# williamyang1991/FRESCO

Measured on AMD Instinct MI355X. Metric: denoising-steps/sec (8-frame batch, 512^2), FRESCO hot-path step, higher is better.
Workload: dtype f16; 1 GPU; cfg2 (BASELINE.json configs[1]): 8 frames 512x512, SD-1.5 decoder shapes, FRESCO attention only (3x up_blocks.2 HW=1024 C=640 + 3x up_blocks.3 HW=4096 C=320 processor calls per step, projections included), 15-step schedule 1x spatial+cf+temporal / 7x cf+temporal / 7x cf; parallelism=single GPU

## Files before the change

fresco_amd/_lib.py:

```python
import ctypes
import os

_HERE = os.path.dirname(os.path.abspath(__file__))
LIB_PATH = os.environ.get("FRESCO_HIP_LIB") or os.path.join(_HERE, "lib", "libfresco_hip.so")

OK = 0
ERRORS = {
    -1: "FRESCO_EINVAL (null pointer / bad size / inconsistent arguments)",
    -2: "FRESCO_EUNSUPPORTED (shape outside what the kernels are built for)",
    -3: "FRESCO_EWORKSPACE (workspace too small)",
    -4: "FRESCO_ELAUNCH (HIP launch failed)",
}
F16, F32, BF16 = 0, 1, 2
VERSION = "0.5.0.2"


class FrescoHipError(RuntimeError):
    pass


_c = ctypes
_vp, _i, _f, _d, _sz, _i64 = _c.c_void_p, _c.c_int, _c.c_float, _c.c_double, _c.c_size_t, _c.c_int64

SIGNATURES = {
    "fresco_version": (_c.c_char_p, []),
    "fresco_last_error": (_c.c_char_p, []),
    "fresco_prof_enable": (_i, [_i]),
    "fresco_prof_disable": (_i, []),
    "fresco_prof_read": (_i, [_i, _vp, _vp, _vp]),
# ... 72 lines not shown
    "fresco_egnet_resize_add": (_i, [_vp] * 5 + [_i] * 7 + [_f, _vp, _vp]),
    "fresco_egnet_saliency": (_i, [_vp, _vp, _vp] + [_i] * 6 + [_vp]),
    "fresco_canny_workspace_bytes": (_sz, [_i, _i, _i]),
    "fresco_canny_classify": (_i, [_vp, _vp, _i, _i, _i, _i, _i, _vp]),
    "fresco_canny_hysteresis": (_i, [_vp, _vp, _vp, _i, _vp, _sz, _i, _i, _i, _vp]),
}

KEYFRAME_SIGNATURES = {
    "keyframe_resize_table_bytes": (_sz, [_i, _i, _i, _i]),
    "keyframe_resize_table": (_i, [_i, _i, _i, _i, _vp, _sz]),
    "keyframe_resize_area_u8": (_i, [_vp, _vp, _vp, _sz, _i, _i, _i, _i, _i, _vp]),
    "keyframe_workspace_bytes": (_sz, [_i, _i, _i]),
    "keyframe_frame_errors": (_i, [_vp, _vp, _vp, _vp, _sz, _i, _i, _i, _vp]),
}

_lib = None


def load():
    global _lib
    if _lib is not None:
        return _lib
    if not os.path.exists(LIB_PATH):
        raise FrescoHipError(
            "fresco_amd: %s is missing -- build it with `python -c 'import __graft_entry__ as g; g.build()'` "
            "or `make -C fresco_amd/csrc`. There is no CPU / eager fallback." % LIB_PATH)
    try:
        lib = ctypes.CDLL(LIB_PATH)
    except OSError as e:
        raise FrescoHipError("fresco_amd: cannot load %s: %s" % (LIB_PATH, e))
    for name, (res, args) in list(SIGNATURES.items()) + list(KEYFRAME_SIGNATURES.items()):
        try:
            fn = getattr(lib, name)
        except AttributeError:
            raise FrescoHipError("fresco_amd: %s does not export %s (stale build?)" % (LIB_PATH, name))
        fn.restype = res
        fn.argtypes = args
    built = lib.fresco_version().decode().split()
    if built[1:2] != [VERSION]:
        raise FrescoHipError("fresco_amd: %s is version %s, this package binds %s (stale build?)"
                             % (LIB_PATH, " ".join(built[1:2]) or "?", VERSION))
    _lib = lib
    return lib


def check(rc, what):
# ... 6 lines not shown
```

fresco_amd/csrc/attn.hip:

```cpp
#include "attn_cfg.h"
#include "lds_dma.h"
#include <type_traits>

namespace fresco {

template <typename T, int D>
__device__ __forceinline__ void kv_pack_body(const T* __restrict__ k, const T* __restrict__ v,
                                             const int32_t* __restrict__ kv_rows, char* __restrict__ img,
                                             float* __restrict__ ktmax, int H, int M, int nT, int64_t group_rows,
                                             int64_t kv_ld) {
    using Cfg = AttnCfg<D>;
    typedef typename Elem<T>::x8 X8;
    const int tile = blockIdx.x, h = blockIdx.y, g = blockIdx.z;
    __shared__ int32_t rows[64];
    __shared__ __attribute__((aligned(16))) T ks[64][D + 8];
    __shared__ __attribute__((aligned(16))) T vs[64][D + 8];

    if (threadIdx.x < 64) {
        const int m = tile * 64 + threadIdx.x;
        int32_t r = -1;
        if (m < M) r = kv_rows ? kv_rows[m] : m;
        rows[threadIdx.x] = r;
    }
    __syncthreads();
// ... 387 lines not shown
                    if (dA + 8 < D) {
                        const u32x2 a = __builtin_bit_cast(u32x2, wa), bb = __builtin_bit_cast(u32x2, wb);
                        const auto s0 = __builtin_amdgcn_permlane32_swap(a[0], bb[0], false, false);
                        const auto s1 = __builtin_amdgcn_permlane32_swap(a[1], bb[1], false, false);
                        u32x4 st;
                        st[0] = s0[0]; st[1] = s1[0]; st[2] = s0[1]; st[3] = s1[1];
                        if (qr < Lq) *reinterpret_cast<u32x4*>(op + dA + hi * 8) = st;
                    } else if (qr < Lq) {
                        *reinterpret_cast<X4*>(op + dA + hi * 4) = wa;
                    }
                }
        }
    }
}

template <int D, int QB>
struct FlashHalves : std::integral_constant<bool, D == 80 && QB == 2> {};

template <typename T, int D, int QB>
__device__ __forceinline__ void flash_body(const T* __restrict__ q, const char* __restrict__ img,
                                           const float* __restrict__ ktmax, T* __restrict__ out, int H, int Lq,
                                           int M, int nT, int batch_per_group, float scale_log2,
                                           float diag_bias_log2, int64_t q_ld, int h, int qblk, int b, int tid) {
    using Cfg = AttnCfg<D>;
    typedef typename Elem<T>::x8 X8;
    constexpr bool FOLD = FoldCfg<T>::ENABLE;
    extern __shared__ __attribute__((aligned(16))) char smem[];
    constexpr int ROWS = 256 * QB;
    const int g = b / batch_per_group;
    const int C = H * D;

    const int lane = tid & 63, wave = tid >> 6;
    const int l31 = lane & 31, hi = lane >> 5;
    const int qrow0 = qblk * ROWS + wave * 32 * QB + l31;
    const int wave_s = __builtin_amdgcn_readfirstlane(wave);
    const int grpB = wave_s >= 4 ? 1 : 0;

    X8 qf[QB][Cfg::NKS];
    float q2[QB];
#pragma unroll
    for (int j = 0; j < QB; ++j) {
        const int qr = qrow0 + 32 * j;
        const T* qp = q + ((int64_t)b * Lq + (qr < Lq ? qr : Lq - 1)) * q_ld + h * D;
        q2[j] = 0.f;
#pragma unroll
        for (int ks = 0; ks < Cfg::NKS; ++ks) {
            const int d0 = ks * 16 + hi * 8;
            X8 t = {0, 0, 0, 0, 0, 0, 0, 0};
            if (d0 < D) t = *reinterpret_cast<const X8*>(qp + d0);
#pragma unroll
            for (int e = 0; e < 8; ++e) q2[j] = fmaf((float)t[e], (float)t[e], q2[j]);
            qf[j][ks] = t;
        }
        q2[j] += __shfl_xor(q2[j], 32, 64);
    }

    float kmax;
    {
        const float* km = ktmax + (int64_t)(g * H + h) * nT;
        float k2 = 0.f;
        for (int i = lane; i < nT; i += 64) k2 = fmaxf(k2, km[i]);
#pragma unroll
        for (int off = 32; off > 0; off >>= 1) k2 = fmaxf(k2, __shfl_xor(k2, off, 64));
        kmax = sqrtf(k2);
// ... 54 lines not shown
#pragma unroll
            for (int r = 0; r < 16; ++r) {
                s[j][0][r] = Cfg::MCOL ? 0.f : negm[j][r];
                s[j][1][r] = Cfg::MCOL ? 0.f : negm[j][r];
            }
#pragma unroll
        for (int ks = 0; ks < Cfg::NKS; ++ks)
#pragma unroll
            for (int kb = 0; kb < 2; ++kb)
#pragma unroll
                for (int j = 0; j < QB; ++j) {
                    s[j][kb] = Elem<T>::mfma32x32x16(kf[kb][ks], qf[j][ks], s[j][kb]);
                }
    };

    ring.stage(0, 3);
    ring.stage(1, 0);
    if (nT > 1) ring.stage(2, 1);
    if (nT > 2) ring.stage(3, 2);
    ring.wait_barrier(nT > 2 ? 2 : (nT > 1 ? 1 : 0));
    {
        X8 kf[2][Cfg::NKS];
        read_k(kf, 3);
        qk(kf);
    }
    __builtin_amdgcn_sched_barrier(0);

    const int need_diag = diag_bias_log2 != 0.f ? 1 : 0;

    int nomax = 0;
    auto step = [&](int u, auto last_c, auto fast_c) __attribute__((always_inline)) {
        constexpr bool LAST = decltype(last_c)::value;
        constexpr bool FAST = decltype(fast_c)::value;
        const int slot = u & 3;
// ... 125 lines not shown
            u = 1;
            if (!need_diag) {
                bool safe = true;
#pragma unroll
                for (int j = 0; j < QB; ++j) safe = safe && (cmul * (qbound[j] - m_run[j]) <= NOMAX_THR);
                nomax = __builtin_amdgcn_readfirstlane((int)__all(safe));
            }
            if (!need_diag)
                for (; u + 3 < nT; ++u) step(u, no_last, fast);
            for (; u < nT - 1; ++u) step(u, no_last, no);
        }
        nomax = 0;
        step(u, yes, no);
    }

    flash_store<T, D, QB>(o, l_run, out, (int64_t)b * Lq, Lq, C, h, qrow0, l31, hi);
}

template <int X>
__device__ __forceinline__ float lane_xor(float v) {
    return __builtin_bit_cast(float, __builtin_amdgcn_ds_swizzle(__builtin_bit_cast(int, v), (X << 10) | 0x1f));
}

template <typename T, int D>
__device__ __forceinline__ void flash_body_halves(const T* __restrict__ q, const char* __restrict__ img,
                                                  const float* __restrict__ ktmax, T* __restrict__ out, int H,
                                                  int Lq, int M, int nT, int batch_per_group, float scale_log2,
                                                  float diag_bias_log2, int64_t q_ld, int h, int qblk, int b) {
    using Cfg = AttnCfg<D>;
    typedef typename Elem<T>::x8 X8;
    constexpr bool FOLD = FoldCfg<T>::ENABLE;
// ... 312 lines not shown
        const int nQblk = (Lq + 256 * QB - 1) / (256 * QB);                                                           \
        const unsigned blk = blockIdx.x;                                                                              \
        const int h = blk % H;                                                                                        \
        const int qblk = (blk / H) % nQblk;                                                                           \
        const int b = blk / (H * nQblk);                                                                              \
        if constexpr (FlashHalves<D, QB>::value)                                                                      \
            flash_body_halves<T, D>(q, img, ktmax, out, H, Lq, M, nT, batch_per_group, scale_log2, diag_bias_log2,     \
                                    q_ld, h, qblk, b);                                                                \
        else                                                                                                          \
            flash_body<T, D, QB>(q, img, ktmax, out, H, Lq, M, nT, batch_per_group, scale_log2, diag_bias_log2, q_ld,  \
                                 h, qblk, b, threadIdx.x);                                                            \
    }
FRESCO_FLASH_KERNEL(attn_flash_kernel, half_t)
FRESCO_FLASH_KERNEL(attn_flash_bf16_kernel, bf16_t)
#undef FRESCO_FLASH_KERNEL

template <typename T, int D, int QB>
static auto flash_kernel_of() {
    if constexpr (std::is_same<T, bf16_t>::value)
        return &attn_flash_bf16_kernel<D, QB>;
    else
        return &attn_flash_kernel<D, QB>;
}
template <typename T, int D>
static auto kv_pack_kernel_of() {
    if constexpr (std::is_same<T, bf16_t>::value)
        return &kv_pack_bf16_kernel<D>;
    else
        return &kv_pack_kernel<D>;
}
// ... 143 lines not shown
    if (workspace_bytes < attn_ws_bytes(n_groups, H, M, D)) return FRESCO_EWORKSPACE;
    hipStream_t st = as_stream(stream);
    char* ws = static_cast<char*>(workspace);
    return with_elem(dtype, [&](auto e) {
        using T = decltype(e);
        const T* qh = static_cast<const T*>(q);
        const T* xh = static_cast<const T*>(x);
        const T* wk = static_cast<const T*>(Wk);
        const T* wv = static_cast<const T*>(Wv);
        T* oh = static_cast<T*>(out);
        if (D == 40)
            return launch_kvproj_attn<T, 320, 40>(qh, xh, x_ld, x_rows, wk, wv, oh, ws, B, H, Lq, n_groups, M, scale, q_ld, st);
        return launch_kvproj_attn<T, 640, 80>(qh, xh, x_ld, x_rows, wk, wv, oh, ws, B, H, Lq, n_groups, M, scale, q_ld, st);
    });
}
```

fresco_amd/csrc/common.hip:

```cpp
#include "common.h"
#include <string.h>
#include <atomic>
#include <map>
#include <mutex>
#include <utility>

namespace fresco {
static thread_local char g_last_error[256] = "";
void set_last_error(hipError_t e) {
    const char* s = hipGetErrorString(e);
    strncpy(g_last_error, s ? s : "unknown HIP error", sizeof(g_last_error) - 1);
    g_last_error[sizeof(g_last_error) - 1] = 0;
}

static std::mutex g_lds_mu;
static std::map<std::pair<const void*, int>, int> g_lds;

int allow_dyn_lds(const void* fn, int bytes) {
    int dev = 0;
    hipError_t e = hipGetDevice(&dev);
    if (e == hipSuccess) {
        std::lock_guard<std::mutex> lock(g_lds_mu);
        int& allowed = g_lds[{fn, dev}];
        if (bytes <= allowed) return FRESCO_OK;
// ... 79 lines not shown
    using namespace fresco;
    int n = g_prof_n < max_records ? g_prof_n : max_records;
    for (int i = 0; i < n; ++i) {
        (void)hipEventSynchronize(g_prof[i].e1);
        float t = 0.f;
        (void)hipEventElapsedTime(&t, g_prof[i].e0, g_prof[i].e1);
        if (tags) tags[i] = g_prof[i].tag;
        if (dims)
            for (int j = 0; j < 4; ++j) dims[i * 4 + j] = g_prof[i].dims[j];
        if (ms) ms[i] = t;
    }
    g_prof_n = 0;
    return n;
}

extern "C" const char* fresco_version(void) { return "fresco_hip 0.5.0.2 gfx950"; }
extern "C" const char* fresco_last_error(void) { return fresco::g_last_error; }
```

fresco_amd/csrc/temporal.hip:

```cpp
#include "common.h"
#include "lds_dma.h"
#include <type_traits>

namespace fresco {

typedef _Float16 half2_t __attribute__((ext_vector_type(2)));


template <typename T, int D, int KT>
__device__ __forceinline__ void temporal_mfma_body(
    const T* __restrict__ q, const T* __restrict__ k, const T* __restrict__ v,
    const int64_t* __restrict__ fwd_map, const uint8_t* __restrict__ mask, T* __restrict__ out,
    int N, int HW, int H, int PB, int chunk, float scale_log2, int64_t q_ld, int64_t k_ld, int64_t v_ld, int packed) {
    typedef typename Elem<T>::x4 X4;
    typedef typename Elem<T>::x8 X8;
    extern __shared__ __attribute__((aligned(16))) char smem[];
    constexpr int NK32 = (D + 31) / 32;
    constexpr int NDT = (D + 15) / 16;
    const int C = H * D;
    const int Hs = H / (int)gridDim.z;
    const int col0 = blockIdx.z * Hs * D;
    const int CC = Hs * D / 8;
    const int RS = 16 * (CC | 1);
    const int c = blockIdx.y;
    const int p0 = blockIdx.x * PB;
    const int tid = threadIdx.x;
    const int NT = blockDim.x;
    const int R = PB * N;
    const int lane = tid & 63;
    const int wave = __builtin_amdgcn_readfirstlane(tid >> 6);
    const int nwaves = NT >> 6;

    char* qs = smem;
// ... 43 lines not shown
    const int ntiles = KT == 1 ? 1 : (N + 15) / 16;
    const int qtr = KT == 1 ? li / N : 0;
    int koff[KT], voff[KT][4], kg[KT][4];
    bool kok[KT][4];
#pragma unroll
    for (int kt = 0; kt < KT; ++kt) {
        koff[kt] = min(kt * 16 + li, R - 1) * RS;
#pragma unroll
        for (int r = 0; r < 4; ++r) {
            const int rel = kt * 16 + 4 * lj + r;
            voff[kt][r] = min(rel, R - 1) * RS;
            kok[kt][r] = rel < R && (KT == 1 ? rel / N == qtr : true);
            kg[kt][r] = KT == 1 ? rel % N : min(rel, N - 1);
        }
    }
    const X4 ones = {(T)1.f, (T)1.f, (T)1.f, (T)1.f};
    const X8 zero8 = {0, 0, 0, 0, 0, 0, 0, 0};

    {
        for (int tb = 0; tb < ntiles; ++tb) {
            const int qr = tb * 16 + li;
            const bool qok = qr < R;
            const int qrow = qok ? qr : R - 1;
            bool ok[KT][4];
#pragma unroll
            for (int kt = 0; kt < KT; ++kt)
#pragma unroll
                for (int r = 0; r < 4; ++r) ok[kt][r] = qok && kok[kt][r] && msk[qrow * N + kg[kt][r]] != 0;
            for (int h = wave; h < Hs; h += nwaves) {
                char* qseg = qs + (size_t)qrow * RS + h * D * 2;
                const char* kh = ks + h * D * 2;
                const char* vh = vs + h * D * 2;
                X8 bq[NK32], ak[KT][NK32];
#pragma unroll
                for (int s = 0; s < NK32; ++s) {
                    const int ch = s * 4 + lj;
                    const X8 tq = *reinterpret_cast<const X8*>(qseg + min(ch, D / 8 - 1) * 16);
                    bq[s] = ch < D / 8 ? tq : zero8;
#pragma unroll
                    for (int kt = 0; kt < KT; ++kt)
                        ak[kt][s] = *reinterpret_cast<const X8*>(kh + koff[kt] + min(ch, D / 8 - 1) * 16);
                }
                X4 av[NDT][KT];
#pragma unroll
                for (int dt = 0; dt < NDT; ++dt) {
                    const int d = min(dt * 16 + li, D - 1);
#pragma unroll
                    for (int kt = 0; kt < KT; ++kt)
#pragma unroll
                        for (int r = 0; r < 4; ++r)
                            av[dt][kt][r] = *reinterpret_cast<const T*>(vh + voff[kt][r] + d * 2);
                }
                float sc[KT][4];
                float m = -INFINITY;
#pragma unroll
                for (int kt = 0; kt < KT; ++kt) {
                    floatx4 acc = {0.f, 0.f, 0.f, 0.f};
#pragma unroll
                    for (int s = 0; s < NK32; ++s)
                        acc = Elem<T>::mfma16x16x32(ak[kt][s], bq[s], acc);
#pragma unroll
                    for (int r = 0; r < 4; ++r) {
                        sc[kt][r] = ok[kt][r] ? acc[r] * scale_log2 : -INFINITY;
                        m = fmaxf(m, sc[kt][r]);
                    }
                }
                m = fmaxf(m, __shfl_xor(m, 16, 64));
                m = fmaxf(m, __shfl_xor(m, 32, 64));
                X4 pb[KT];
#pragma unroll
                for (int kt = 0; kt < KT; ++kt)
#pragma unroll
                    for (int r = 0; r < 4; ++r) pb[kt][r] = (T)__builtin_amdgcn_exp2f(sc[kt][r] - m);
                floatx4 den = {0.f, 0.f, 0.f, 0.f};
#pragma unroll
                for (int kt = 0; kt < KT; ++kt)
                    den = Elem<T>::mfma16x16x16(ones, pb[kt], den);
                floatx4 o[NDT];
#pragma unroll
                for (int dt = 0; dt < NDT; ++dt) {
                    o[dt] = floatx4{0.f, 0.f, 0.f, 0.f};
#pragma unroll
                    for (int kt = 0; kt < KT; ++kt)
                        o[dt] = Elem<T>::mfma16x16x16(av[dt][kt], pb[kt], o[dt]);
                }
                const float inv = __builtin_amdgcn_rcpf(den[0]);
                if (qok) {
#pragma unroll
                    for (int dt = 0; dt < NDT; ++dt) {
                        const int d0 = dt * 16 + 4 * lj;
                        if (d0 < D) {
                            X4 ov;
#pragma unroll
                            for (int r = 0; r < 4; ++r) ov[r] = (T)(o[dt][r] * inv);
                            *reinterpret_cast<X4*>(qseg + d0 * 2) = ov;
                        }
                    }
                }
            }
        }
        __syncthreads();

        for (int r = wave; r < R; r += nwaves) {
            const int ro = __builtin_amdgcn_readfirstlane(rows[r]);
            if (ro < 0) continue;
            T* dst = out + (int64_t)ro * C + col0;
            for (int part = 0; part < ppr; ++part) {
                const int cc = part * 64 + lane;
                if (cc < CC)
                    *reinterpret_cast<uint4*>(dst + cc * 8) =
                        *reinterpret_cast<const uint4*>(qs + (size_t)r * RS + cc * 16);
            }
        }
// ... 344 lines not shown
```

fresco_amd/ops.py:

```python
import ctypes
import math

import torch

from . import _lib
from ._lib import FrescoHipError


try:
    _raw_stream = torch._C._cuda_getCurrentRawStream
except AttributeError:
    _raw_stream = None


def _stream():
    if _raw_stream is not None:
        return _raw_stream(torch.cuda.current_device())
    return torch.cuda.current_stream().cuda_stream


def _need_gpu(*tensors):
    for t in tensors:
        if t is not None and not t.is_cuda:
            raise FrescoHipError("fresco_amd operators run on the GPU only (got a %s tensor); "
# ... 574 lines not shown
        fwd_map = fwd_map.to(torch.int64)
    return fwd_map.contiguous()


def _prep_maps(fwd_map, mask, N, HW):
    if fwd_map is not None:
        fwd_map = _prep_fwd_map(fwd_map, N, HW)
    mask = mask.reshape(-1, N, N)
    if mask.dtype == torch.bool:
        mask = mask.contiguous().view(torch.uint8)
    elif mask.dtype != torch.uint8:
        mask = (mask != 0).contiguous().view(torch.uint8)
    return fwd_map, mask.contiguous()


def temporal_attention(q, k, v, fwd_map, mask, heads, scale, chunk):
    _need_gpu(q, k, v, fwd_map, mask)
    if q.dtype not in _MFMA_DTYPES or k.dtype != q.dtype or v.dtype != q.dtype:
        raise TypeError("fresco_amd.temporal_attention: q, k, v must all be fp16 or all bf16 (got %s/%s/%s)"
                        % (q.dtype, k.dtype, v.dtype))
    Bt, HW, C = q.shape
    N = Bt // chunk
    D = C // heads
    q, q_ld, _ = _rows(q)
    k, k_ld, _ = _rows(k)
    v, v_ld, _ = _rows(v)
    owner = fwd_map
    fwd_map, mask = _prep_maps(fwd_map, mask, N, HW)
    _check_permutations(owner, fwd_map, HW)
    out = torch.empty((Bt, HW, C), dtype=q.dtype, device=q.device)
# ... 612 lines not shown
```

fresco_amd/processor.py:

```python
import math
import warnings
import weakref

import torch

from . import _lib, ops
from .control import AttentionControl


def _plain_linear(m, with_bias, nw=1):
    return (type(m) is torch.nn.Linear and (m.bias is not None) == with_bias and m.weight.is_cuda
            and ops.linear_supported(m.in_features, m.out_features, m.weight.dtype, nw))


class FRESCOAttnProcessor2_0:
    def __init__(self, unet_chunk_size=2, controller=None):
        _lib.load()
        self.unet_chunk_size = unet_chunk_size
        self.controller = controller
        self._ws = ops.Workspace()
        self._rows_cache = {}
        self.shard = None
        self.fuse_projections = True
        self.sparse_kv_projection = True
        self.fuse_kv_pack = True

    native_bf16 = True
    fuse_kv_pack_bf16 = False

    def _kernel_dtype(self, dtype):
        return dtype == torch.float16 or (dtype == torch.bfloat16 and self.native_bf16)

    def _project(self, attn, x, names, outs=None, x_rows=None):
        mods = [getattr(attn, n) for n in names]
        if (self.fuse_projections and self._kernel_dtype(x.dtype) and x.is_cuda
                and all(_plain_linear(m, False, len(mods)) and m.weight.dtype == x.dtype for m in mods)
                and (outs is None or all(o.dtype == x.dtype for o in outs))
                and len({(m.in_features, m.out_features) for m in mods}) == 1
                and all(m.weight.is_contiguous() and m.weight.data_ptr() % 16 == 0 for m in mods)):
            return ops.linear(x, [m.weight.detach() for m in mods], None, outs, x_rows=x_rows, x_rows_trusted=True)
        if x_rows is not None:
            x = x.reshape(-1, x.shape[-1]).index_select(0, x_rows.long())
        res = [m(x) for m in mods]
# ... 74 lines not shown
            raise NotImplementedError("fresco_amd: attention_mask with head dim %d (no larger kernel head dim)" % D)

        def pad(x, L, col):
            xp = x.new_zeros(B, L, heads, Dp)
            xp[..., :D] = x.view(B, L, heads, D)
            if col is not None:
                xp[..., D] = col
            return xp.view(B, L, heads * Dp)

        bias = bias.clamp_min(-5.0e4 * scale)
        qp = pad(q, Lq, 1.0 / scale)
        kp = pad(k, Lk, bias.transpose(1, 2).to(k.dtype))
        vp = pad(v, Lk, None)
        out = ops.attention(qp, kp, vp, heads, scale, workspace=self._ws)
        return out.view(B, Lq, heads, Dp)[..., :D].reshape(B, Lq, C)

    def _cf_mask(self, ctrl, hw):
        mask = None
        if ctrl.attn_mask is not None:
            for m in ctrl.attn_mask:
                if m.shape[1] == hw:
                    mask = m
        return mask

    def __call__(self, attn, hidden_states, encoder_hidden_states=None, attention_mask=None, temb=None):
        residual = hidden_states
        if attn.spatial_norm is not None:
            hidden_states = attn.spatial_norm(hidden_states, temb)
        input_ndim = hidden_states.ndim
        if input_ndim == 4:
# ... 76 lines not shown
        head_dim = query.shape[-1] // heads
        sm_scale = 1.0 / math.sqrt(head_dim)
        fresco = bool(ctrl) and not crossattn
        chunk = self.unet_chunk_size

        q_att = query
        if fresco and ctrl.use_intraattn:
            ref = ctrl(None)
            assert ref.shape == encoder_hidden_states.shape
            q_ref, k_ref = self._project(attn, ref, ("to_q", "to_k"))
            if q_ref.dtype != query.dtype:
                q_ref, k_ref = q_ref.to(query.dtype), k_ref.to(query.dtype)
            q_att = ops.attention(q_ref, k_ref, query, heads, ctrl.intraattn_scale_factor * sm_scale,
                                  diag_bias=float(ctrl.intraattn_bias), workspace=self._ws)

        if mask_bias is not None:
            if fresco and ctrl.use_cfattn:
                if self._cf_mask(ctrl, key.shape[1]) is not None or sparse_kv:
                    raise ValueError("fresco_amd: attention_mask cannot be combined with the masked cross-frame key set "
                                     "(the mask addresses %d keys, the cross-frame pass has another key set)" % mask_bias.shape[-1])
                nf = key.shape[0] // chunk
                k0 = key.view(chunk, nf, key.shape[1], -1)[:, :1].expand(-1, nf, -1, -1).reshape(key.shape)
                v0 = value.view(chunk, nf, value.shape[1], -1)[:, :1].expand(-1, nf, -1, -1).reshape(value.shape)
                hs = self._masked_attention(q_att, k0, v0, heads, sm_scale, mask_bias)
            else:
                hs = self._masked_attention(q_att, key, value, heads, sm_scale, mask_bias)
        elif fresco and ctrl.use_cfattn and fused_kv is not None:
            hs = ops.attention_kvproj(q_att, hidden_states, fused_kv[0], fused_kv[1], fused_kv[2], heads, sm_scale,
                                      n_groups=chunk, M=fused_kv[3], workspace=self._ws)
        elif fresco and ctrl.use_cfattn and sparse_kv:
            hs = ops.attention(q_att, key, value, heads, sm_scale, n_groups=chunk, M=key.shape[1],
                               group_rows=key.shape[1], workspace=self._ws)
        elif fresco and ctrl.use_cfattn:
            video_length = key.shape[0] // chunk
            hw = key.shape[1]
            mask = self._cf_mask(ctrl, hw)
            rows = self._kv_rows(mask) if mask is not None else None
            hs = ops.attention(q_att, key, value, heads, sm_scale, kv_rows=rows, n_groups=chunk,
                               M=hw if rows is None else rows.numel(), group_rows=video_length * hw,
                               workspace=self._ws)
        else:
            hs = ops.attention(q_att, key, value, heads, sm_scale, workspace=self._ws)

        if fresco and ctrl.use_interattn:
            fwd_mapping = interattn_mask = None
            paras = ctrl.interattn_paras
            for i, f in enumerate(paras["fwd_mappings"]):
                if f.shape[2] == hs.shape[1]:
                    fwd_mapping = f
                    interattn_mask = paras["interattn_masks"][i]
            if fwd_mapping is None:
                raise ValueError("fresco_amd: no temporal-attention parameters for %d tokens" % hs.shape[1])
            hs = ops.temporal_attention(query, key, hs, fwd_mapping, interattn_mask, heads,
                                        ctrl.interattn_scale_factor * sm_scale, chunk)

        hs = hs.to(out_dtype)
        hs = self._project_out(attn, hs)
        hs = attn.to_out[1](hs)
        if input_ndim == 4:
            hs = hs.transpose(-1, -2).reshape(batch_size, channel, height, width)
        if attn.residual_connection:
            hs = hs + residual
        if attn.rescale_output_factor != 1.0:
            hs = hs / attn.rescale_output_factor
        return hs


# ... 80 lines not shown
```

include/fresco_hip.h:

```cpp
#ifndef FRESCO_HIP_H
#define FRESCO_HIP_H

#include <stddef.h>
#include <stdint.h>

#ifdef __cplusplus
extern "C" {
#endif

#define FRESCO_OK 0
#define FRESCO_EINVAL (-1)
#define FRESCO_EUNSUPPORTED (-2)
#define FRESCO_EWORKSPACE (-3)
#define FRESCO_ELAUNCH (-4)

#define FRESCO_F16 0
#define FRESCO_F32 1
#define FRESCO_BF16 2

const char* fresco_version(void);
const char* fresco_last_error(void);

#define FRESCO_PROF_ATTN_FLASH 1
#define FRESCO_PROF_KV_PACK 2
#define FRESCO_PROF_TEMPORAL 3
#define FRESCO_PROF_OPT_TSIGN 4
#define FRESCO_PROF_OPT_TGRAD 5
#define FRESCO_PROF_OPT_COLNORM 6
#define FRESCO_PROF_OPT_GRAM 7
#define FRESCO_PROF_OPT_SV 8
#define FRESCO_PROF_OPT_ADAM 9
#define FRESCO_PROF_LINEAR 10
#define FRESCO_PROF_ATTN_F32 11
#define FRESCO_PROF_FN_GEMM 12
#define FRESCO_PROF_EBSYNTH_LEVEL 13
int fresco_prof_enable(int capacity);
int fresco_prof_disable(void);
int fresco_prof_read(int max_records, int* tags, int* dims, float* ms);

size_t fresco_attn_workspace_bytes(int n_groups, int H, int M, int D);
int fresco_attn_fwd(const void* q, const void* k, const void* v, const int32_t* kv_rows,
                    void* out, void* workspace, size_t workspace_bytes,
                    int B, int H, int Lq, int D,
                    int n_groups, int M, int64_t group_rows,
                    float scale, float diag_bias, int64_t q_ld, int64_t kv_ld, int dtype, void* stream);

int fresco_linear(const void* x, int64_t x_ld, const int32_t* x_rows, const void* W0, const void* W1, const void* W2,
                  const void* b0, const void* b1, const void* b2, void* out0, void* out1, void* out2, int64_t ld0,
                  int64_t ld1, int64_t ld2, int nw, int M, int N, int K, int dtype, void* stream);

// ... 206 lines not shown
```

Baseline: 495.7 denoising-steps/sec.

## Fuse temporal attention into the kv-projected cross-frame flash attention epilogue

Adds a flash attention kernel variant whose queries are gathered in trajectory order (via the forward mapping), so each block holds whole per-pixel frame groups. After softmax normalization, the epilogue runs temporal attention across the frames in LDS and scatters the result back to the original rows. This removes the separate temporal pack, attention and unpack launches and their HBM round trips. In exchange the kernel uses more LDS per block, does gathered query loads, and is limited to f16 with D=40 (the up_blocks.3 layers).

```diff
diff --git a/fresco_amd/_lib.py b/fresco_amd/_lib.py
--- a/fresco_amd/_lib.py
+++ b/fresco_amd/_lib.py
@@ -12,7 +12,7 @@
     -4: "FRESCO_ELAUNCH (HIP launch failed)",
 }
 F16, F32, BF16 = 0, 1, 2
-VERSION = "0.5.0.2"
+VERSION = "0.5.0.3"
 
 
 class FrescoHipError(RuntimeError):
@@ -115,6 +115,12 @@
     "keyframe_frame_errors": (_i, [_vp, _vp, _vp, _vp, _sz, _i, _i, _i, _vp]),
 }
 
+ATTN_TEMPORAL_SIGNATURES = {
+    "attn_temporal_supported": (_i, [_i] * 6),
+    "attn_temporal_fwd_kvproj": (_i, [_vp, _vp, _i64, _vp, _vp, _vp, _vp, _vp, _sz, _i, _i, _i, _i, _i, _i, _i, _f, _i64, _i,
+                                      _vp, _i64, _vp, _i64, _vp, _vp, _f, _i, _vp]),
+}
+
 _lib = None
 
 
@@ -130,7 +136,7 @@
         lib = ctypes.CDLL(LIB_PATH)
     except OSError as e:
         raise FrescoHipError("fresco_amd: cannot load %s: %s" % (LIB_PATH, e))
-    for name, (res, args) in list(SIGNATURES.items()) + list(KEYFRAME_SIGNATURES.items()):
+    for name, (res, args) in list(SIGNATURES.items()) + list(KEYFRAME_SIGNATURES.items()) + list(ATTN_TEMPORAL_SIGNATURES.items()):
         try:
             fn = getattr(lib, name)
         except AttributeError:
diff --git a/fresco_amd/csrc/attn.hip b/fresco_amd/csrc/attn.hip
--- a/fresco_amd/csrc/attn.hip
+++ b/fresco_amd/csrc/attn.hip
@@ -1,5 +1,6 @@
 #include "attn_cfg.h"
 #include "lds_dma.h"
+#include "temporal_unit.h"
 #include <type_traits>
 
 namespace fresco {
@@ -425,14 +426,116 @@
     }
 }
 
+template <typename T>
+struct TrajArgs {
+    const T* tq;
+    const T* tk;
+    const int64_t* fwd_map;
+    const uint8_t* mask;
+    float tscale_log2;
+    int N;
+    int64_t tq_ld, tk_ld;
+};
+
+template <int D, int QB>
+struct TrajLds {
+    static constexpr int RS = 16 * ((D / 8) | 1);
+    static constexpr int WROWS = 32 * QB;
+    static constexpr int Q_OFF = AttnCfg<D>::LDS_BYTES;
+    static constexpr int K_OFF = Q_OFF + 8 * WROWS * RS;
+    static constexpr int V_OFF = K_OFF + 8 * WROWS * RS;
+    static constexpr int ROWS_OFF = V_OFF + 8 * 32 * RS;
+    static constexpr int MASK_OFF = ROWS_OFF + 8 * WROWS * 4;
+    static constexpr int LDS_BYTES = MASK_OFF + 8 * WROWS * 2;
+};
+
+template <typename T, int D, int QB>
+__device__ __forceinline__ void flash_temporal_epilogue(const floatx16 (&o)[QB][AttnCfg<D>::NDB], const float (&l_run)[QB],
+                                                        T* __restrict__ out, const TrajArgs<T>& ta, char* smem, int C,
+                                                        int HW, int h, int qblk) {
+    using Cfg = AttnCfg<D>;
+    using TL = TrajLds<D, QB>;
+    typedef typename Elem<T>::x4 X4;
+    constexpr int RS = TL::RS;
+    int tid = threadIdx.x;
+    asm volatile("" : "+v"(tid));
+    const int lane = tid & 63, wave = __builtin_amdgcn_readfirstlane(tid >> 6);
+    const int l31 = lane & 31, hi = lane >> 5, li = lane & 15, lj = lane >> 4;
+    char* tqs = smem + TL::Q_OFF + wave * (TL::WROWS * RS);
+    const char* tks = smem + TL::K_OFF + wave * (TL::WROWS * RS);
+    char* tvs = smem + TL::V_OFF + wave * (32 * RS);
+    const int* trows = reinterpret_cast<const int*>(smem + TL::ROWS_OFF) + wave * TL::WROWS;
+    const uint16_t* mbits = reinterpret_cast<const uint16_t*>(smem + TL::MASK_OFF) + wave * TL::WROWS;
+    const int N = ta.N, nsh = __builtin_ctz(N);
+    const int qtr = li >> nsh;
+    const int koff[1] = {li * RS};
+    int voff[1][4], kg[4];
+    bool kok[4];
+#pragma unroll
+    for (int r = 0; r < 4; ++r) {
+        const int rel = 4 * lj + r;
+        voff[0][r] = rel * RS;
+        kok[r] = (rel >> nsh) == qtr;
+        kg[r] = rel & (N - 1);
+    }
+#pragma unroll
+    for (int j = 0; j < QB; ++j) {
+        float l_tot;
+        if (Cfg::ONES) {
+            constexpr int rr = D % 32;
+            l_tot = __shfl(o[j][D / 32][(rr & 3) + 4 * (rr >> 3)], l31 + 32 * ((rr >> 2) & 1), 64);
+        } else {
+            l_tot = l_run[j] + __shfl_xor(l_run[j], 32, 64);
+        }
+        const float inv = 1.f / l_tot;
+#pragma unroll
+        for (int db = 0; db < Cfg::NDB; ++db)
+#pragma unroll
+            for (int g4 = 0; g4 < 4; ++g4) {
+                if (db * 32 + g4 * 8 >= D) continue;
+                X4 w;
+#pragma unroll
+                for (int jj = 0; jj < 4; ++jj) w[jj] = (T)(o[j][db][g4 * 4 + jj] * inv);
+                *reinterpret_cast<X4*>(tvs + l31 * RS + (db * 32 + g4 * 8 + 4 * hi) * 2) = w;
+            }
+        asm volatile("s_waitcnt lgkmcnt(0)" ::: "memory");
+        __builtin_amdgcn_wave_barrier();
+#pragma unroll
+        for (int t = 0; t < 2; ++t) {
+            const int trow = 32 * j + 16 * t;
+            const int i0 = qblk * (256 * QB) + wave * TL::WROWS + trow + li;
+            const bool qok = i0 < HW * N;
+            const unsigned mb = mbits[trow + li];
+            bool ok[1][4];
+#pragma unroll
+            for (int r = 0; r < 4; ++r) ok[0][r] = qok && kok[r] && ((mb >> kg[r]) & 1u) != 0;
+            temporal_unit<T, D, 1>(tqs + (trow + li) * RS, tks + trow * RS, tvs + 16 * t * RS, koff, voff, ok, qok,
+                                   ta.tscale_log2, li, lj);
+        }
+        asm volatile("s_waitcnt lgkmcnt(0)" ::: "memory");
+        __builtin_amdgcn_wave_barrier();
+    }
+    constexpr int CPS = D / 8;
+#pragma unroll
+    for (int c0 = 0; c0 < TL::WROWS * CPS; c0 += 64) {
+        const int c = c0 + lane;
+        const int row = min(c / CPS, TL::WROWS - 1), ch = c % CPS;
+        const int gr = trows[row];
+        if (c < TL::WROWS * CPS && gr >= 0)
+            *reinterpret_cast<uint4*>(out + (int64_t)gr * C + h * D + ch * 8) =
+                *reinterpret_cast<const uint4*>(tqs + row * RS + ch * 16);
+    }
+}
+
 template <int D, int QB>
 struct FlashHalves : std::integral_constant<bool, D == 80 && QB == 2> {};
 
-template <typename T, int D, int QB>
+template <typename T, int D, int QB, bool TRAJ = false>
 __device__ __forceinline__ void flash_body(const T* __restrict__ q, const char* __restrict__ img,
                                            const float* __restrict__ ktmax, T* __restrict__ out, int H, int Lq,
                                            int M, int nT, int batch_per_group, float scale_log2,
-                                           float diag_bias_log2, int64_t q_ld, int h, int qblk, int b, int tid) {
+                                           float diag_bias_log2, int64_t q_ld, int h, int qblk, int b, int tid,
+                                           const TrajArgs<T>& ta = TrajArgs<T>()) {
     using Cfg = AttnCfg<D>;
     typedef typename Elem<T>::x8 X8;
     constexpr bool FOLD = FoldCfg<T>::ENABLE;
@@ -447,18 +550,73 @@
     const int wave_s = __builtin_amdgcn_readfirstlane(wave);
     const int grpB = wave_s >= 4 ? 1 : 0;
 
+    if constexpr (TRAJ) {
+        const PackRing<D> ring0(img, g, H, h, nT, smem, wave_s, tid);
+        ring0.stage(0, 3);
+        ring0.stage(1, 0);
+        if (nT > 1) ring0.stage(2, 1);
+        if (nT > 2) ring0.stage(3, 2);
+    }
     X8 qf[QB][Cfg::NKS];
     float q2[QB];
+    const bool same_q = TRAJ && ta.tq == q && ta.tq_ld == q_ld;
 #pragma unroll
     for (int j = 0; j < QB; ++j) {
         const int qr = qrow0 + 32 * j;
-        const T* qp = q + ((int64_t)b * Lq + (qr < Lq ? qr : Lq - 1)) * q_ld + h * D;
+        const T* qp;
+        int64_t grow = 0;
+        if constexpr (TRAJ) {
+            const int pi = qblk * ROWS + wave * 32 * QB + 32 * j + l31;
+            const int p = pi >> __builtin_ctz(ta.N), f = pi & (ta.N - 1);
+            int row = (int)ta.fwd_map[(int64_t)f * Lq + min(p, Lq - 1)];
+            row = min(max(row, 0), Lq - 1);
+            grow = ((int64_t)b + f) * Lq + row;
+            qp = q + grow * q_ld + h * D;
+            if (hi == 0) {
+                const int wr = wave * 32 * QB + 32 * j + l31;
+                reinterpret_cast<int*>(smem + TrajLds<D, QB>::ROWS_OFF)[wr] = p < Lq ? (int)grow : -1;
+                uint32_t mw[4] = {0u, 0u, 0u, 0u};
+                if (p < Lq) {
+                    const uint8_t* mp = ta.mask + (int64_t)pi * ta.N;
+                    if (ta.N == 16) {
+                        const uint4 v4 = *reinterpret_cast<const uint4*>(mp);
+                        mw[0] = v4.x; mw[1] = v4.y; mw[2] = v4.z; mw[3] = v4.w;
+                    } else if (ta.N == 8) {
+                        const uint2 v2 = *reinterpret_cast<const uint2*>(mp);
+                        mw[0] = v2.x; mw[1] = v2.y;
+                    } else if (ta.N == 4) {
+                        mw[0] = *reinterpret_cast<const uint32_t*>(mp);
+                    } else if (ta.N == 2) {
+                        mw[0] = *reinterpret_cast<const uint16_t*>(mp);
+                    } else {
+                        mw[0] = *mp;
+                    }
+                }
+                unsigned bits = 0;
+#pragma unroll
+                for (int e = 0; e < 16; ++e) bits |= ((mw[e >> 2] >> (8 * (e & 3))) & 0xffu) != 0 ? (1u << e) : 0u;
+                reinterpret_cast<uint16_t*>(smem + TrajLds<D, QB>::MASK_OFF)[wr] = (uint16_t)bits;
+            }
+        } else {
+            qp = q + ((int64_t)b * Lq + (qr < Lq ? qr : Lq - 1)) * q_ld + h * D;
+        }
         q2[j] = 0.f;
 #pragma unroll
         for (int ks = 0; ks < Cfg::NKS; ++ks) {
             const int d0 = ks * 16 + hi * 8;
             X8 t = {0, 0, 0, 0, 0, 0, 0, 0};
             if (d0 < D) t = *reinterpret_cast<const X8*>(qp + d0);
+            if constexpr (TRAJ) {
+                using TL = TrajLds<D, QB>;
+                if (d0 < D) {
+                    const int lo = (wave * TL::WROWS + 32 * j + l31) * TL::RS + d0 * 2;
+                    X8 tqv = t;
+                    if (!same_q) tqv = *reinterpret_cast<const X8*>(ta.tq + grow * ta.tq_ld + h * D + d0);
+                    *reinterpret_cast<X8*>(smem + TL::Q_OFF + lo) = tqv;
+                    *reinterpret_cast<X8*>(smem + TL::K_OFF + lo) =
+                        *reinterpret_cast<const X8*>(ta.tk + grow * ta.tk_ld + h * D + d0);
+                }
+            }
 #pragma unroll
             for (int e = 0; e < 8; ++e) q2[j] = fmaf((float)t[e], (float)t[e], q2[j]);
             qf[j][ks] = t;
@@ -543,10 +701,12 @@
                 }
     };
 
-    ring.stage(0, 3);
-    ring.stage(1, 0);
-    if (nT > 1) ring.stage(2, 1);
-    if (nT > 2) ring.stage(3, 2);
+    if constexpr (!TRAJ) {
+        ring.stage(0, 3);
+        ring.stage(1, 0);
+        if (nT > 1) ring.stage(2, 1);
+        if (nT > 2) ring.stage(3, 2);
+    }
     ring.wait_barrier(nT > 2 ? 2 : (nT > 1 ? 1 : 0));
     {
         X8 kf[2][Cfg::NKS];
@@ -702,7 +862,10 @@
         step(u, yes, no);
     }
 
-    flash_store<T, D, QB>(o, l_run, out, (int64_t)b * Lq, Lq, C, h, qrow0, l31, hi);
+    if constexpr (TRAJ)
+        flash_temporal_epilogue<T, D, QB>(o, l_run, out, ta, smem, C, Lq, h, qblk);
+    else
+        flash_store<T, D, QB>(o, l_run, out, (int64_t)b * Lq, Lq, C, h, qrow0, l31, hi);
 }
 
 template <int X>
@@ -1045,6 +1208,22 @@
 FRESCO_FLASH_KERNEL(attn_flash_kernel, half_t)
 FRESCO_FLASH_KERNEL(attn_flash_bf16_kernel, bf16_t)
 #undef FRESCO_FLASH_KERNEL
+
+template <int D, int QB>
+__global__ __launch_bounds__(512, 2) void attn_flash_temporal_kernel(const half_t* __restrict__ q,
+                                                                     const char* __restrict__ img,
+                                                                     const float* __restrict__ ktmax,
+                                                                     half_t* __restrict__ out, int H, int HW, int M,
+                                                                     int nT, float scale_log2, int64_t q_ld,
+                                                                     TrajArgs<half_t> ta) {
+    const int nQblk = (int)(((int64_t)HW * ta.N + 256 * QB - 1) / (256 * QB));
+    const unsigned blk = blockIdx.x;
+    const int h = blk % H;
+    const int qblk = (blk / H) % nQblk;
+    const int g = blk / (H * nQblk);
+    flash_body<half_t, D, QB, true>(q, img, ktmax, out, H, HW, M, nT, ta.N, scale_log2, 0.f, q_ld, h, qblk, g * ta.N,
+                                    threadIdx.x, ta);
+}
 
 template <typename T, int D, int QB>
 static auto flash_kernel_of() {
@@ -1218,3 +1397,75 @@
         return launch_kvproj_attn<T, 640, 80>(qh, xh, x_ld, x_rows, wk, wv, oh, ws, B, H, Lq, n_groups, M, scale, q_ld, st);
     });
 }
+
+#include "../../include/fresco_attn_temporal.h"
+
+namespace fresco {
+template <int KIN, int D>
+static int launch_kvproj_attn_temporal(const half_t* q, const half_t* x, int64_t x_ld, const int32_t* x_rows,
+                                       const half_t* Wk, const half_t* Wv, half_t* out, char* ws, int B, int H, int HW,
+                                       int n_groups, int M, float scale, int64_t q_ld, const TrajArgs<half_t>& ta,
+                                       hipStream_t st) {
+    using Cfg = AttnCfg<D>;
+    const int nT = ntiles_of(M);
+    char* img = ws;
+    float* ktmax = reinterpret_cast<float*>(ws + align_up((size_t)n_groups * H * (nT + 1) * Cfg::TILE, 256));
+    {
+        ProfScope ps(FRESCO_PROF_KV_PACK, n_groups, H, M, -D, st);
+        constexpr int lds = KvProjCfg<KIN, D>::LDS_BYTES;
+        const auto kern = kvproj_pack_kernel_of<half_t, KIN, D>();
+        if (int rc = allow_dyn_lds(kern, lds)) return rc;
+        constexpr int TL = KvProjCfg<KIN, D>::TILES;
+        hipLaunchKernelGGL(kern, dim3((nT + TL - 1) / TL, 2 * (H * D / 160), n_groups), dim3(320), lds, st, x, x_ld, x_rows,
+                           Wk, Wv, img, ktmax, H, M, nT);
+    }
+    constexpr int lds = TrajLds<D, 2>::LDS_BYTES;
+    static_assert(lds <= 160 * 1024, "ring + the waves' q, k, V rows and row tables: one CU's LDS");
+    const auto kern = &attn_flash_temporal_kernel<D, 2>;
+    if (int rc = allow_dyn_lds(kern, lds)) return rc;
+    const int nQblk = (int)(((int64_t)HW * ta.N + 511) / 512);
+    ProfScope ps(FRESCO_PROF_ATTN_TEMPORAL, B * H, HW, M, D, st);
+    hipLaunchKernelGGL(kern, dim3(H * nQblk * n_groups), dim3(512), lds, st, q, img, ktmax, out, H, HW, M, nT,
+                       scale * 1.4426950408889634f, q_ld, ta);
+    return check_launch();
+}
+}
+
+extern "C" int attn_temporal_supported(int H, int D, int K_in, int N, int HW, int dtype) {
+    if (dtype != FRESCO_F16 || !fresco_attn_kvproj_supported(H, D, K_in)) return 0;
+    if (D != 40) return 0;
+    if (!(N == 1 || N == 2 || N == 4 || N == 8 || N == 16) || HW <= 0) return 0;
+    return 1;
+}
+
+extern "C" int attn_temporal_fwd_kvproj(const void* q, const void* x, int64_t x_ld, const int32_t* x_rows, const void* Wk,
+                                        const void* Wv, void* out, void* workspace, size_t workspace_bytes, int B, int H,
+                                        int Lq, int D, int n_groups, int M, int K_in, float scale, int64_t q_ld, int dtype,
+                                        const void* tq, int64_t tq_ld, const void* tk, int64_t tk_ld,
+                                        const int64_t* fwd_map, const uint8_t* mask, float temporal_scale, int N,
+                                        void* stream) {
+    if (dtype != FRESCO_F16 && dtype != FRESCO_BF16) return FRESCO_EINVAL;
+    if (!q || !x || !x_rows || !Wk || !Wv || !out || !workspace || !tq || !tk || !fwd_map || !mask) return FRESCO_EINVAL;
+    if (B <= 0 || H <= 0 || Lq <= 0 || D <= 0 || n_groups <= 0 || M <= 0 || K_in <= 0 || N <= 0) return FRESCO_EINVAL;
+    if (B != n_groups * N || !(scale > 0.f)) return FRESCO_EINVAL;
+    const int64_t Cw = (int64_t)H * D;
+    if (q_ld < Cw || q_ld % 8 != 0 || x_ld < K_in || x_ld % 8 != 0) return FRESCO_EINVAL;
+    if (tq_ld < Cw || tq_ld % 8 != 0 || tk_ld < Cw || tk_ld % 8 != 0) return FRESCO_EINVAL;
+    if (reinterpret_cast<uintptr_t>(mask) % 16 != 0) return FRESCO_EINVAL;
+    if (!attn_temporal_supported(H, D, K_in, N, Lq, dtype)) return FRESCO_EUNSUPPORTED;
+    if ((int64_t)B * Lq + 512 > 0x7fffffff) return FRESCO_EUNSUPPORTED;
+    if (workspace_bytes < attn_ws_bytes(n_groups, H, M, D)) return FRESCO_EWORKSPACE;
+    TrajArgs<half_t> ta;
+    ta.tq = static_cast<const half_t*>(tq);
+    ta.tk = static_cast<const half_t*>(tk);
+    ta.fwd_map = fwd_map;
+    ta.mask = mask;
+    ta.tscale_log2 = temporal_scale * 1.4426950408889634f;
+    ta.N = N;
+    ta.tq_ld = tq_ld;
+    ta.tk_ld = tk_ld;
+    return launch_kvproj_attn_temporal<320, 40>(static_cast<const half_t*>(q), static_cast<const half_t*>(x), x_ld, x_rows,
+                                                static_cast<const half_t*>(Wk), static_cast<const half_t*>(Wv),
+                                                static_cast<half_t*>(out), static_cast<char*>(workspace), B, H, Lq,
+                                                n_groups, M, scale, q_ld, ta, as_stream(stream));
+}
diff --git a/fresco_amd/csrc/common.hip b/fresco_amd/csrc/common.hip
--- a/fresco_amd/csrc/common.hip
+++ b/fresco_amd/csrc/common.hip
@@ -117,5 +117,5 @@
     return n;
 }
 
-extern "C" const char* fresco_version(void) { return "fresco_hip 0.5.0.2 gfx950"; }
+extern "C" const char* fresco_version(void) { return "fresco_hip 0.5.0.3 gfx950"; }
 extern "C" const char* fresco_last_error(void) { return fresco::g_last_error; }
diff --git a/fresco_amd/csrc/temporal.hip b/fresco_amd/csrc/temporal.hip
--- a/fresco_amd/csrc/temporal.hip
+++ b/fresco_amd/csrc/temporal.hip
@@ -1,5 +1,6 @@
 #include "common.h"
 #include "lds_dma.h"
+#include "temporal_unit.h"
 #include <type_traits>
 
 namespace fresco {
@@ -12,11 +13,7 @@
     const T* __restrict__ q, const T* __restrict__ k, const T* __restrict__ v,
     const int64_t* __restrict__ fwd_map, const uint8_t* __restrict__ mask, T* __restrict__ out,
     int N, int HW, int H, int PB, int chunk, float scale_log2, int64_t q_ld, int64_t k_ld, int64_t v_ld, int packed) {
-    typedef typename Elem<T>::x4 X4;
-    typedef typename Elem<T>::x8 X8;
     extern __shared__ __attribute__((aligned(16))) char smem[];
-    constexpr int NK32 = (D + 31) / 32;
-    constexpr int NDT = (D + 15) / 16;
     const int C = H * D;
     const int Hs = H / (int)gridDim.z;
     const int col0 = blockIdx.z * Hs * D;
@@ -90,8 +87,6 @@
             kg[kt][r] = KT == 1 ? rel % N : min(rel, N - 1);
         }
     }
-    const X4 ones = {(T)1.f, (T)1.f, (T)1.f, (T)1.f};
-    const X8 zero8 = {0, 0, 0, 0, 0, 0, 0, 0};
 
     {
         for (int tb = 0; tb < ntiles; ++tb) {
@@ -107,72 +102,7 @@
                 char* qseg = qs + (size_t)qrow * RS + h * D * 2;
                 const char* kh = ks + h * D * 2;
                 const char* vh = vs + h * D * 2;
-                X8 bq[NK32], ak[KT][NK32];
-#pragma unroll
-                for (int s = 0; s < NK32; ++s) {
-                    const int ch = s * 4 + lj;
-                    const X8 tq = *reinterpret_cast<const X8*>(qseg + min(ch, D / 8 - 1) * 16);
-                    bq[s] = ch < D / 8 ? tq : zero8;
-#pragma unroll
-                    for (int kt = 0; kt < KT; ++kt)
-                        ak[kt][s] = *reinterpret_cast<const X8*>(kh + koff[kt] + min(ch, D / 8 - 1) * 16);
-                }
-                X4 av[NDT][KT];
-#pragma unroll
-                for (int dt = 0; dt < NDT; ++dt) {
-                    const int d = min(dt * 16 + li, D - 1);
-#pragma unroll
-                    for (int kt = 0; kt < KT; ++kt)
-#pragma unroll
-                        for (int r = 0; r < 4; ++r)
-                            av[dt][kt][r] = *reinterpret_cast<const T*>(vh + voff[kt][r] + d * 2);
-                }
-                float sc[KT][4];
-                float m = -INFINITY;
-#pragma unroll
-                for (int kt = 0; kt < KT; ++kt) {
-                    floatx4 acc = {0.f, 0.f, 0.f, 0.f};
-#pragma unroll
-                    for (int s = 0; s < NK32; ++s)
-                        acc = Elem<T>::mfma16x16x32(ak[kt][s], bq[s], acc);
-#pragma unroll
-                    for (int r = 0; r < 4; ++r) {
-                        sc[kt][r] = ok[kt][r] ? acc[r] * scale_log2 : -INFINITY;
-                        m = fmaxf(m, sc[kt][r]);
-                    }
-                }
-                m = fmaxf(m, __shfl_xor(m, 16, 64));
-                m = fmaxf(m, __shfl_xor(m, 32, 64));
-                X4 pb[KT];
-#pragma unroll
-                for (int kt = 0; kt < KT; ++kt)
-#pragma unroll
-                    for (int r = 0; r < 4; ++r) pb[kt][r] = (T)__builtin_amdgcn_exp2f(sc[kt][r] - m);
-                floatx4 den = {0.f, 0.f, 0.f, 0.f};
-#pragma unroll
-                for (int kt = 0; kt < KT; ++kt)
-                    den = Elem<T>::mfma16x16x16(ones, pb[kt], den);
-                floatx4 o[NDT];
-#pragma unroll
-                for (int dt = 0; dt < NDT; ++dt) {
-                    o[dt] = floatx4{0.f, 0.f, 0.f, 0.f};
-#pragma unroll
-                    for (int kt = 0; kt < KT; ++kt)
-                        o[dt] = Elem<T>::mfma16x16x16(av[dt][kt], pb[kt], o[dt]);
-                }
-                const float inv = __builtin_amdgcn_rcpf(den[0]);
-                if (qok) {
-#pragma unroll
-                    for (int dt = 0; dt < NDT; ++dt) {
-                        const int d0 = dt * 16 + 4 * lj;
-                        if (d0 < D) {
-                            X4 ov;
-#pragma unroll
-                            for (int r = 0; r < 4; ++r) ov[r] = (T)(o[dt][r] * inv);
-                            *reinterpret_cast<X4*>(qseg + d0 * 2) = ov;
-                        }
-                    }
-                }
+                temporal_unit<T, D, KT>(qseg, kh, vh, koff, voff, ok, qok, scale_log2, li, lj);
             }
         }
         __syncthreads();
diff --git a/fresco_amd/csrc/temporal_unit.h b/fresco_amd/csrc/temporal_unit.h
--- /dev/null
+++ b/fresco_amd/csrc/temporal_unit.h
@@ -0,0 +1,84 @@
+#pragma once
+#include "common.h"
+
+namespace fresco {
+
+template <typename T, int D, int KT>
+__device__ __forceinline__ void temporal_unit(char* qseg, const char* kh, const char* vh, const int (&koff)[KT],
+                                              const int (&voff)[KT][4], const bool (&ok)[KT][4], bool qok,
+                                              float scale_log2, int li, int lj) {
+    typedef typename Elem<T>::x4 X4;
+    typedef typename Elem<T>::x8 X8;
+    constexpr int NK32 = (D + 31) / 32;
+    constexpr int NDT = (D + 15) / 16;
+    const X4 ones = {(T)1.f, (T)1.f, (T)1.f, (T)1.f};
+    const X8 zero8 = {0, 0, 0, 0, 0, 0, 0, 0};
+    X8 bq[NK32], ak[KT][NK32];
+#pragma unroll
+    for (int s = 0; s < NK32; ++s) {
+        const int ch = s * 4 + lj;
+        const X8 tq = *reinterpret_cast<const X8*>(qseg + min(ch, D / 8 - 1) * 16);
+        bq[s] = ch < D / 8 ? tq : zero8;
+#pragma unroll
+        for (int kt = 0; kt < KT; ++kt)
+            ak[kt][s] = *reinterpret_cast<const X8*>(kh + koff[kt] + min(ch, D / 8 - 1) * 16);
+    }
+    X4 av[NDT][KT];
+#pragma unroll
+    for (int dt = 0; dt < NDT; ++dt) {
+        const int d = min(dt * 16 + li, D - 1);
+#pragma unroll
+        for (int kt = 0; kt < KT; ++kt)
+#pragma unroll
+            for (int r = 0; r < 4; ++r)
+                av[dt][kt][r] = *reinterpret_cast<const T*>(vh + voff[kt][r] + d * 2);
+    }
+    float sc[KT][4];
+    float m = -INFINITY;
+#pragma unroll
+    for (int kt = 0; kt < KT; ++kt) {
+        floatx4 acc = {0.f, 0.f, 0.f, 0.f};
+#pragma unroll
+        for (int s = 0; s < NK32; ++s)
+            acc = Elem<T>::mfma16x16x32(ak[kt][s], bq[s], acc);
+#pragma unroll
+        for (int r = 0; r < 4; ++r) {
+            sc[kt][r] = ok[kt][r] ? acc[r] * scale_log2 : -INFINITY;
+            m = fmaxf(m, sc[kt][r]);
+        }
+    }
+    m = fmaxf(m, __shfl_xor(m, 16, 64));
+    m = fmaxf(m, __shfl_xor(m, 32, 64));
+    X4 pb[KT];
+#pragma unroll
+    for (int kt = 0; kt < KT; ++kt)
+#pragma unroll
+        for (int r = 0; r < 4; ++r) pb[kt][r] = (T)__builtin_amdgcn_exp2f(sc[kt][r] - m);
+    floatx4 den = {0.f, 0.f, 0.f, 0.f};
+#pragma unroll
+    for (int kt = 0; kt < KT; ++kt)
+        den = Elem<T>::mfma16x16x16(ones, pb[kt], den);
+    floatx4 o[NDT];
+#pragma unroll
+    for (int dt = 0; dt < NDT; ++dt) {
+        o[dt] = floatx4{0.f, 0.f, 0.f, 0.f};
+#pragma unroll
+        for (int kt = 0; kt < KT; ++kt)
+            o[dt] = Elem<T>::mfma16x16x16(av[dt][kt], pb[kt], o[dt]);
+    }
+    const float inv = __builtin_amdgcn_rcpf(den[0]);
+    if (qok) {
+#pragma unroll
+        for (int dt = 0; dt < NDT; ++dt) {
+            const int d0 = dt * 16 + 4 * lj;
+            if (d0 < D) {
+                X4 ov;
+#pragma unroll
+                for (int r = 0; r < 4; ++r) ov[r] = (T)(o[dt][r] * inv);
+                *reinterpret_cast<X4*>(qseg + d0 * 2) = ov;
+            }
+        }
+    }
+}
+
+}
diff --git a/fresco_amd/ops.py b/fresco_amd/ops.py
--- a/fresco_amd/ops.py
+++ b/fresco_amd/ops.py
@@ -612,6 +612,56 @@
     return fwd_map, mask.contiguous()
 
 
+def attention_kvproj_temporal_supported(heads, head_dim, in_features, N, HW, dtype):
+    if dtype not in _MFMA_DTYPES:
+        return False
+    return bool(_lib.load().attn_temporal_supported(int(heads), int(head_dim), int(in_features), int(N), int(HW),
+                                                    _MFMA_DTYPES[dtype]))
+
+
+def attention_kvproj_temporal(q, hidden, x_rows, w_k, w_v, heads, scale, n_groups, M, tq, tk, fwd_map, mask,
+                              temporal_scale, workspace=None):
+    _need_gpu(q, hidden, x_rows, w_k, w_v, tq, tk, fwd_map, mask)
+    dt = q.dtype
+    if dt not in _MFMA_DTYPES or any(t.dtype != dt for t in (hidden, w_k, w_v, tq, tk)) or x_rows.dtype != torch.int32:
+        raise TypeError("fresco_amd.attention_kvproj_temporal: q, hidden, w_k, w_v, tq, tk of one MFMA dtype and an int32 row "
+                        "table required (got %s/%s/%s/%s/%s/%s, %s)"
+                        % (q.dtype, hidden.dtype, w_k.dtype, w_v.dtype, tq.dtype, tk.dtype, x_rows.dtype))
+    B, HW, C = q.shape
+    D = C // heads
+    K_in = hidden.shape[-1]
+    N = B // n_groups
+    if tq.shape != q.shape or tk.shape != q.shape or N * n_groups != B:
+        raise ValueError("attention_kvproj_temporal: tq, tk must have q's shape %s, a multiple of n_groups batch rows"
+                         % (tuple(q.shape),))
+    if w_k.shape != (C, K_in) or w_v.shape != (C, K_in) or not (w_k.is_contiguous() and w_v.is_contiguous()):
+        raise ValueError("attention_kvproj_temporal: contiguous (%d, %d) weights expected" % (C, K_in))
+    if x_rows.numel() != n_groups * M or not x_rows.is_contiguous():
+        raise ValueError("attention_kvproj_temporal: x_rows must hold n_groups * M = %d entries" % (n_groups * M))
+    q, q_ld, _ = _rows(q)
+    tq, tq_ld, _ = _rows(tq)
+    tk, tk_ld, _ = _rows(tk)
+    hidden, x_ld, _ = _rows(hidden)
+    owner = fwd_map
+    fwd_map, mask = _prep_maps(fwd_map, mask, N, HW)
+    _check_permutations(owner, fwd_map, HW)
+    if mask.shape[0] != HW:
+        raise ValueError("attention_kvproj_temporal: mask must be (%d, %d, %d)" % (HW, N, N))
+    if mask.data_ptr() % 16:
+        mask = mask.clone()
+    lib = _lib.load()
+    ws_bytes = lib.fresco_attn_workspace_bytes(n_groups, heads, M, D)
+    ws = (workspace or _default_ws).get(ws_bytes, q.device)
+    out = torch.empty((B, HW, C), dtype=dt, device=q.device)
+    rc = lib.attn_temporal_fwd_kvproj(q.data_ptr(), hidden.data_ptr(), x_ld, x_rows.data_ptr(), w_k.data_ptr(),
+                                      w_v.data_ptr(), out.data_ptr(), ws.data_ptr(), ws.numel(), B, heads, HW, D, n_groups,
+                                      M, K_in, float(scale), q_ld, _MFMA_DTYPES[dt], tq.data_ptr(), tq_ld, tk.data_ptr(),
+                                      tk_ld, fwd_map.data_ptr(), mask.data_ptr(), float(temporal_scale), N, _stream())
+    _lib.check(rc, "attn_temporal_fwd_kvproj(B=%d,H=%d,HW=%d,D=%d,groups=%d,M=%d,K=%d,N=%d)"
+               % (B, heads, HW, D, n_groups, M, K_in, N))
+    return out
+
+
 def temporal_attention(q, k, v, fwd_map, mask, heads, scale, chunk):
     _need_gpu(q, k, v, fwd_map, mask)
     if q.dtype not in _MFMA_DTYPES or k.dtype != q.dtype or v.dtype != q.dtype:
diff --git a/fresco_amd/processor.py b/fresco_amd/processor.py
--- a/fresco_amd/processor.py
+++ b/fresco_amd/processor.py
@@ -27,6 +27,7 @@
 
     native_bf16 = True
     fuse_kv_pack_bf16 = False
+    fuse_temporal = True
 
     def _kernel_dtype(self, dtype):
         return dtype == torch.float16 or (dtype == torch.bfloat16 and self.native_bf16)
@@ -131,6 +132,18 @@
         vp = pad(v, Lk, None)
         out = ops.attention(qp, kp, vp, heads, scale, workspace=self._ws)
         return out.view(B, Lq, heads, Dp)[..., :D].reshape(B, Lq, C)
+
+    @staticmethod
+    def _temporal_paras(ctrl, hw):
+        fwd_mapping = interattn_mask = None
+        paras = ctrl.interattn_paras
+        for i, f in enumerate(paras["fwd_mappings"]):
+            if f.shape[2] == hw:
+                fwd_mapping = f
+                interattn_mask = paras["interattn_masks"][i]
+        if fwd_mapping is None:
+            raise ValueError("fresco_amd: no temporal-attention parameters for %d tokens" % hw)
+        return fwd_mapping, interattn_mask
 
     def _cf_mask(self, ctrl, hw):
         mask = None
@@ -237,6 +250,7 @@
             q_att = ops.attention(q_ref, k_ref, query, heads, ctrl.intraattn_scale_factor * sm_scale,
                                   diag_bias=float(ctrl.intraattn_bias), workspace=self._ws)
 
+        temporal_done = False
         if mask_bias is not None:
             if fresco and ctrl.use_cfattn:
                 if self._cf_mask(ctrl, key.shape[1]) is not None or sparse_kv:
@@ -249,8 +263,17 @@
             else:
                 hs = self._masked_attention(q_att, key, value, heads, sm_scale, mask_bias)
         elif fresco and ctrl.use_cfattn and fused_kv is not None:
-            hs = ops.attention_kvproj(q_att, hidden_states, fused_kv[0], fused_kv[1], fused_kv[2], heads, sm_scale,
-                                      n_groups=chunk, M=fused_kv[3], workspace=self._ws)
+            if (ctrl.use_interattn and self.fuse_temporal and q_att.dtype == query.dtype == key.dtype
+                    and ops.attention_kvproj_temporal_supported(heads, head_dim, hidden_states.shape[-1],
+                                                                q_att.shape[0] // chunk, q_att.shape[1], q_att.dtype)):
+                fwd_mapping, interattn_mask = self._temporal_paras(ctrl, q_att.shape[1])
+                hs = ops.attention_kvproj_temporal(q_att, hidden_states, fused_kv[0], fused_kv[1], fused_kv[2], heads,
+                                                   sm_scale, chunk, fused_kv[3], query, key, fwd_mapping, interattn_mask,
+                                                   ctrl.interattn_scale_factor * sm_scale, workspace=self._ws)
+                temporal_done = True
+            else:
+                hs = ops.attention_kvproj(q_att, hidden_states, fused_kv[0], fused_kv[1], fused_kv[2], heads, sm_scale,
+                                          n_groups=chunk, M=fused_kv[3], workspace=self._ws)
         elif fresco and ctrl.use_cfattn and sparse_kv:
             hs = ops.attention(q_att, key, value, heads, sm_scale, n_groups=chunk, M=key.shape[1],
                                group_rows=key.shape[1], workspace=self._ws)
@@ -265,15 +288,8 @@
         else:
             hs = ops.attention(q_att, key, value, heads, sm_scale, workspace=self._ws)
 
-        if fresco and ctrl.use_interattn:
-            fwd_mapping = interattn_mask = None
-            paras = ctrl.interattn_paras
-            for i, f in enumerate(paras["fwd_mappings"]):
-                if f.shape[2] == hs.shape[1]:
-                    fwd_mapping = f
-                    interattn_mask = paras["interattn_masks"][i]
-            if fwd_mapping is None:
-                raise ValueError("fresco_amd: no temporal-attention parameters for %d tokens" % hs.shape[1])
+        if fresco and ctrl.use_interattn and not temporal_done:
+            fwd_mapping, interattn_mask = self._temporal_paras(ctrl, hs.shape[1])
             hs = ops.temporal_attention(query, key, hs, fwd_mapping, interattn_mask, heads,
                                         ctrl.interattn_scale_factor * sm_scale, chunk)
 
diff --git a/include/fresco_attn_temporal.h b/include/fresco_attn_temporal.h
--- /dev/null
+++ b/include/fresco_attn_temporal.h
@@ -0,0 +1,21 @@
+#ifndef FRESCO_ATTN_TEMPORAL_H
+#define FRESCO_ATTN_TEMPORAL_H
+
+#include <stddef.h>
+#include <stdint.h>
+
+#ifdef __cplusplus
+extern "C" {
+#endif
+
+int attn_temporal_supported(int H, int D, int K_in, int N, int HW, int dtype);
+int attn_temporal_fwd_kvproj(const void* q, const void* x, int64_t x_ld, const int32_t* x_rows, const void* Wk,
+                             const void* Wv, void* out, void* workspace, size_t workspace_bytes, int B, int H, int Lq,
+                             int D, int n_groups, int M, int K_in, float scale, int64_t q_ld, int dtype, const void* tq,
+                             int64_t tq_ld, const void* tk, int64_t tk_ld, const int64_t* fwd_map, const uint8_t* mask,
+                             float temporal_scale, int N, void* stream);
+
+#ifdef __cplusplus
+}
+#endif
+#endif
diff --git a/include/fresco_hip.h b/include/fresco_hip.h
--- a/include/fresco_hip.h
+++ b/include/fresco_hip.h
@@ -34,6 +34,7 @@
 #define FRESCO_PROF_ATTN_F32 11
 #define FRESCO_PROF_FN_GEMM 12
 #define FRESCO_PROF_EBSYNTH_LEVEL 13
+#define FRESCO_PROF_ATTN_TEMPORAL 14
 int fresco_prof_enable(int capacity);
 int fresco_prof_disable(void);
 int fresco_prof_read(int max_records, int* tags, int* dims, float* ms);
```

After: 498.3 denoising-steps/sec (median of 6 runs). No clear change (+0.5%).
